# abstractqqq/polars_ds_extension

Measured on AMD Instinct MI355X. Metric: grouped lstsq regressions/sec (1e8 rows x 16 f64 feats; Gram-build GB/s under gram_build), higher is better.
Workload: dtype f64; 1 GPU; group_by(key).agg(lin_reg): 1000000 groups x 100 rows x 16 f64 feats of the frame (1e+08 rows), OLS with rank gate (pl_lr default path), inputs resident in HBM; `value`: the groups given as row offsets (pre-segmented, as Polars hands groups to pl_lr -- the cpu_baseline gets the same); the same step starting from a sorted int64 key column: grouped_by_key; groups_total=1000000, groups_per_gpu=1000000, rows_per_group=100, features=16, parallelism=group-sharded x1

## Files before the change

polars_ds_extension_amd/csrc/grouped_fused.hip:

```cpp
#include <type_traits>

#include "moments_dev.hpp"
#include "solve_reg_dev.hpp"

namespace pds {

#ifdef PDS_PROFILE_PHASES
__device__ unsigned long long g_phase_cycles[8];
#define PDS_T0() const unsigned long long _t0 = __builtin_amdgcn_s_memtime()
#define PDS_T1(k) prof[k] += __builtin_amdgcn_s_memtime() - _t0
#else
#define PDS_T0() do {} while (0)
#define PDS_T1(k) do {} while (0)
#endif

constexpr int kFQ = 18;
constexpr int kFM = kFQ * kFQ;
constexpr int kFTile = 17 * kColStride;
constexpr int kFWaveLds = kFTile + kFM * 8;

template <typename T, bool BIAS>
__device__ __forceinline__ void consume_range(const char* wl, int lane, int rel0, int rel1, WaveAcc& a) {
    const int f = lane & 15, q = lane >> 4;
    const T* xcol = reinterpret_cast<const T*>(wl + f * kColStride) + q;
    const T* ycol = reinterpret_cast<const T*>(wl + kSlotY * kColStride) + q;
    int s0 = rel0 >> 2;
    const int s1 = (rel1 + 3) >> 2;
    using Acc = typename Tile<T>::acc;
    Acc acc;
    double xy, cs, yy, ys;
    if constexpr (sizeof(T) == 8) {
        acc = Acc{a.d[0], a.d[1], a.d[2], a.d[3]};
        xy = a.xy; cs = a.cs; yy = a.yy; ys = a.ys;
    } else {
        acc = Acc{0, 0, 0, 0};
        xy = cs = yy = ys = 0.0;
    }
    T fxy = 0, fcs = 0, fyy = 0, fys = 0;
    auto step_v = [&](T x, T yv) __attribute__((always_inline)) {
        acc = Tile<T>::mfma(x, x, acc);
        if constexpr (sizeof(T) == 8) {
            xy = fma(x, yv, xy);
            if constexpr (BIAS) {
                cs += x;
                ys += yv;
            }
        } else {
            fxy = fmaf(x, yv, fxy);
            if constexpr (BIAS) {
                fcs += x;
                fys += yv;
            }
        }
    };
    auto step = [&](int s, bool masked, int lo, int hi) __attribute__((always_inline)) {
        T x = xcol[4 * s];
        T yv = ycol[4 * s];
        if (masked) {
            const bool in = q >= lo && q < hi;
            x = in ? x : T(0);
            yv = in ? yv : T(0);
        }
        acc = Tile<T>::mfma(x, x, acc);
        if constexpr (sizeof(T) == 8) {
            xy = fma(x, yv, xy);
            if constexpr (BIAS) {
                cs += x;
                ys += yv;
            }
        } else {
            fxy = fmaf(x, yv, fxy);
            if constexpr (BIAS) {
                fcs += x;
                fys += yv;
            }
        }
    };
    if (rel0 & 3) {
        const int lo = rel0 & 3;
        const int hi = min(rel1 - 4 * s0, 4);
        step(s0, true, lo, hi);
        ++s0;
    }
    const int sfull = rel1 >> 2;
    int s = s0;
    for (; s + 4 <= sfull; s += 4) {
        const T x0 = xcol[4 * s], x1 = xcol[4 * s + 4], x2 = xcol[4 * s + 8], x3 = xcol[4 * s + 12];
        const T y0 = ycol[4 * s], y1 = ycol[4 * s + 4], y2 = ycol[4 * s + 8], y3 = ycol[4 * s + 12];
        step_v(x0, y0);
        step_v(x1, y1);
        step_v(x2, y2);
        step_v(x3, y3);
    }
    for (; s < sfull; ++s) step_v(xcol[4 * s], ycol[4 * s]);
    if ((rel1 & 3) && sfull >= s0 && sfull < s1) step(sfull, true, 0, rel1 & 3);
    if constexpr (sizeof(T) == 8) {
        a.d[0] = acc[0]; a.d[1] = acc[1]; a.d[2] = acc[2]; a.d[3] = acc[3];
        a.xy = xy; a.cs = cs; a.yy = yy; a.ys = ys;
    } else {
        a.d[0] += (double)acc[0]; a.d[1] += (double)acc[1]; a.d[2] += (double)acc[2]; a.d[3] += (double)acc[3];
        a.xy += (double)fxy; a.cs += (double)fcs; a.yy += (double)fyy; a.ys += (double)fys;
    }
}

template <typename T, bool BIAS>
__device__ __forceinline__ void consume_range_pack(const char* wl, int lane, int rel0, int rel1, WaveAcc& a) {
    const int f = lane & 15, q = lane >> 4;
    const int roff = q + 4 * (f >> 3);
    const T* xcol = reinterpret_cast<const T*>(wl + (f & 7) * kColStride) + roff;
    const T* ycol = reinterpret_cast<const T*>(wl + kSlotY * kColStride) + roff;
    int s0 = rel0 >> 3;
    const int s1 = (rel1 + 7) >> 3;
    using Acc = typename Tile<T>::acc;
    Acc acc;
    double xy, cs, yy, ys;
    if constexpr (sizeof(T) == 8) {
        acc = Acc{a.d[0], a.d[1], a.d[2], a.d[3]};
        xy = a.xy; cs = a.cs; yy = a.yy; ys = a.ys;
    } else {
        acc = Acc{0, 0, 0, 0};
        xy = cs = yy = ys = 0.0;
    }
    T fxy = 0, fcs = 0, fyy = 0, fys = 0;
    auto step_v = [&](T x, T yv) __attribute__((always_inline)) {
        acc = Tile<T>::mfma(x, x, acc);
        if constexpr (sizeof(T) == 8) {
            xy = fma(x, yv, xy);
            if constexpr (BIAS) {
                cs += x;
                ys += yv;
            }
        } else {
            fxy = fmaf(x, yv, fxy);
            if constexpr (BIAS) {
                fcs += x;
                fys += yv;
            }
        }
    };
    auto step_m = [&](int s) __attribute__((always_inline)) {
        const int r = 8 * s + roff;
        const bool in = r >= rel0 && r < rel1;
        const T x = in ? xcol[8 * s] : T(0);
        const T yv = in ? ycol[8 * s] : T(0);
        step_v(x, yv);
    };
    if (rel0 & 7) {
        step_m(s0);
        ++s0;
    }
    const int sfull = rel1 >> 3;
    int s = s0;
    for (; s + 4 <= sfull; s += 4) {
        const T x0 = xcol[8 * s], x1 = xcol[8 * s + 8], x2 = xcol[8 * s + 16], x3 = xcol[8 * s + 24];
        const T y0 = ycol[8 * s], y1 = ycol[8 * s + 8], y2 = ycol[8 * s + 16], y3 = ycol[8 * s + 24];
        step_v(x0, y0);
        step_v(x1, y1);
        step_v(x2, y2);
        step_v(x3, y3);
    }
    for (; s < sfull; ++s) step_v(xcol[8 * s], ycol[8 * s]);
    if ((rel1 & 7) && sfull >= s0 && sfull < s1) step_m(sfull);
    if constexpr (sizeof(T) == 8) {
        a.d[0] = acc[0]; a.d[1] = acc[1]; a.d[2] = acc[2]; a.d[3] = acc[3];
        a.xy = xy; a.cs = cs; a.yy = yy; a.ys = ys;
    } else {
        a.d[0] += (double)acc[0]; a.d[1] += (double)acc[1]; a.d[2] += (double)acc[2]; a.d[3] += (double)acc[3];
        a.xy += (double)fxy; a.cs += (double)fcs; a.yy += (double)fyy; a.ys += (double)fys;
    }
}

__device__ __forceinline__ int64_t lower_bound_i64(const int64_t* __restrict__ a, int64_t n, int64_t key) {
    int64_t lo = 0, hi = n;
    while (lo < hi) {
        const int64_t mid = (lo + hi) >> 1;
        if (a[mid] < key) lo = mid + 1;
        else hi = mid;
    }
    return lo;
}

template <typename T, int LPS, bool CHOL, bool BIAS, int PC>
__global__ __launch_bounds__(64) void grouped_stream_kernel(const T* const* __restrict__ cols, int p_arg,
                                                            const int64_t* __restrict__ offsets, int64_t n_groups,
                                                            int64_t n_rows, SolveRegDev sp, T* __restrict__ coeffs,
                                                            uint8_t* __restrict__ flags, int32_t* __restrict__ mark_list,
                                                            unsigned* __restrict__ mark_count, unsigned* __restrict__ mark_host_flag) {
    constexpr int SPW = 64 / LPS;
    constexpr int RPL = Tile<T>::RPL;
    constexpr int TR = 64 * RPL;
    constexpr int NA = CHOL ? LPS + 1 : LPS;
    constexpr bool PACK = LPS <= 8;
    constexpr int ZSLOT = PACK ? 7 : 15;
    extern __shared__ __attribute__((aligned(16))) char smem[];
    const int lane = threadIdx.x & 63;
    char* wl = smem;
    double* Msc = reinterpret_cast<double*>(smem + kFTile);
    constexpr bool FULLP = PC != 0;
    static_assert(PC >= 0 && PC <= LPS, "PC is a feature count of this kernel size");
    const int p = FULLP ? PC : p_arg;
    const int pp = p;
    const int pout = p + (BIAS ? 1 : 0);
    const int sub = lane / LPS, j_in = lane % LPS;

    const int64_t W = gridDim.x, w = blockIdx.x;
    const int64_t base_row = offsets[0];
    const int64_t total = offsets[n_groups] - base_row;
    const int64_t gl = (w == 0) ? 0 : lower_bound_i64(offsets, n_groups, base_row + (total * w) / W);
    const int64_t gh = (w == W - 1) ? n_groups : lower_bound_i64(offsets, n_groups, base_row + (total * (w + 1)) / W);
    if (gl >= gh) return;
    const int64_t rlo = offsets[gl], rhi = offsets[gh];

    {
        typename Tile<T>::vec z;
#pragma unroll
        for (int e = 0; e < RPL; ++e) z[e] = T(0);
        for (int c = p; c < 16; ++c) *reinterpret_cast<typename Tile<T>::vec*>(wl + c * kColStride + lane * 16) = z;
    }
#ifdef PDS_PROFILE_PHASES
    unsigned long long prof[8] = {0, 0, 0, 0, 0, 0, 0, 0};
    const unsigned long long t_begin = __builtin_amdgcn_s_memtime();
#endif
    double a_p[NA];
    double b_p[CHOL ? 1 : LPS];
    double dj_p = 1.0;
    double cs_p = 0.0, ys_p = 0.0, n_p = 1.0;
    bool null_p = false;
    int npend = 0;
    int64_t gbase = gl;

    auto solve_pending = [&]() __attribute__((always_inline)) {
        int j = j_in;
        asm volatile("" : "+v"(j));
        const bool colv = j < pp;
        const int64_t sys = gbase + sub;
        const bool live = sub < npend;
        const bool few = null_p;
        bool is_null = null_p;
        bool suspect = false;
        double zj = 0.0;
        int pj = j;
        PDS_T0();
        if constexpr (CHOL) {
            SolveRegDev spk = sp;
            spk.pp = p;
            spk.p = spk.pp;
            spk.gate_on = 1;
            chol_core<LPS>(a_p, dj_p, j, spk, is_null, zj, &suspect);
            suspect = suspect && !few;
            is_null = is_null || suspect;
        } else {
            solve_core<LPS>(a_p, b_p, dj_p, j, lane, sp, is_null, pj, zj);
        }
        if (live && colv) coeffs[sys * (int64_t)pout + pj] = is_null ? (T)__builtin_nan("") : (T)zj;
        if constexpr (BIAS) {
            const double sb = Grp<LPS>::sum(colv ? cs_p * zj : 0.0);
            const double b0 = (ys_p - sb) / n_p;
            if (live && j == 0) coeffs[sys * (int64_t)pout + p] = is_null ? (T)__builtin_nan("") : (T)b0;
        }
        if (live && j == 0 && flags) flags[sys] = suspect ? 2 : (is_null ? 1 : 0);
        if constexpr (CHOL) {
            const bool mk = suspect && live && j == 0;
            const unsigned long long mm = __ballot(mk);
            if (mm != 0ull && mark_list) {
                const int leader = __ffsll((long long)mm) - 1;
                unsigned slot = 0;
                if (lane == leader) {
                    slot = atomicAdd(mark_count, (unsigned)__popcll(mm));
                    __hip_atomic_store(mark_host_flag, 1u, __ATOMIC_RELAXED, __HIP_MEMORY_SCOPE_SYSTEM);
                }
                slot = __shfl(slot, leader);
                if (mk) mark_list[slot + __popcll(mm & ((1ull << lane) - 1ull))] = (int32_t)sys;
            }
        }
        PDS_T1(3);
        gbase += npend;
        npend = 0;
    };

    WaveAcc acc;
    zero_acc(acc);
    int64_t g = gl;
    int64_t gs = rlo;
    int64_t ge = offsets[g + 1];
    uint32_t g_left = (uint32_t)(gh - gl);
    int64_t ge_next = offsets[g_left >= 2 ? g + 2 : gh];
    int64_t pos = rlo;

    auto flush_group = [&]() __attribute__((always_inline)) {
        PDS_T0();
        const uint64_t ng = (uint64_t)(ge - gs);
        const bool too_few = (uint32_t)(ng >> 32) == 0u && (uint32_t)ng < (uint32_t)pout;
        {
            const int jj = lane & 15;
            constexpr bool RFOLD = PACK && sizeof(T) == 8;
            auto shl8 = [](double v) __attribute__((always_inline)) {
                int lo = __double2loint(v), hi = __double2hiint(v);
                lo = __builtin_amdgcn_update_dpp(0, lo, 0x108 , 0xf, 0xf, true);
                hi = __builtin_amdgcn_update_dpp(0, hi, 0x108, 0xf, 0xf, true);
                return __hiloint2double(hi, lo);
            };
            if constexpr (RFOLD) {
                const double d0 = acc.d[0] + shl8(acc.d[2]), d1 = acc.d[1] + shl8(acc.d[3]);
                if (jj < 8) {
                    Msc[Tile<T>::drow(lane, 0) + kFQ * jj] = d0;
                    Msc[Tile<T>::drow(lane, 1) + kFQ * jj] = d1;
                }
            } else {
#pragma unroll
                for (int r = 0; r < 4; ++r) Msc[Tile<T>::drow(lane, r) + kFQ * jj] = acc.d[r];
            }
            double xy = xor_sum_q(acc.xy);
            if constexpr (RFOLD) xy += shl8(xy);
            if (lane < (RFOLD ? 8 : 16)) Msc[lane + kFQ * 17] = xy;
            if constexpr (BIAS) {
                double cs = xor_sum_q(acc.cs), ys = xor_sum_q(acc.ys);
                if constexpr (RFOLD) {
                    cs += shl8(cs);
                    ys += shl8(ys);
                }
                if (lane < (RFOLD ? 8 : 16)) Msc[lane + kFQ * 16] = cs;
                if (lane == 0) {
                    Msc[16 + kFQ * 16] = (double)ng;
                    Msc[16 + kFQ * 17] = ys;
                }
                if (PACK && !RFOLD && lane == 8) Msc[17 + kFQ * 17] = ys;
            }
        }
        if constexpr (PACK && sizeof(T) != 8) {
            PDS_WAVE_LDS_SYNC();
            const int fi = lane & 7, fj = lane >> 3;
            const double dsum = Msc[fi + kFQ * fj] + Msc[fi + 8 + kFQ * (fj + 8)];
            double xys = 0.0, css = 0.0, yss = 0.0;
            if (lane < 8) {
                xys = Msc[lane + kFQ * 17] + Msc[lane + 8 + kFQ * 17];
                if constexpr (BIAS) css = Msc[lane + kFQ * 16] + Msc[lane + 8 + kFQ * 16];
            }
            if (BIAS && lane == 0) yss = Msc[16 + kFQ * 17] + Msc[17 + kFQ * 17];
            PDS_WAVE_LDS_SYNC();
            Msc[fi + kFQ * fj] = dsum;
            if (lane < 8) {
                Msc[lane + kFQ * 17] = xys;
                if constexpr (BIAS) Msc[lane + kFQ * 16] = css;
            }
            if (BIAS && lane == 0) Msc[16 + kFQ * 17] = yss;
        }
        if (sp.lambda > 0.0) {
            PDS_WAVE_LDS_SYNC();
            if (lane < p) Msc[lane * (kFQ + 1)] += sp.lambda;
        }
        PDS_WAVE_LDS_SYNC();
        {
            int j = j_in;
            asm volatile("" : "+v"(j));
            const int lj = (j < p) ? j : ZSLOT;
            if (sub == npend) {
                const double* colp = Msc + kFQ * lj;
                if (p >= LPS) {
#pragma unroll
                    for (int i = 0; i < LPS; ++i) {
                        a_p[i] = colp[i];
                        if constexpr (!CHOL) b_p[i] = Msc[i + kFQ * 17];
                    }
                } else {
#pragma unroll
                    for (int i = 0; i < LPS; ++i) {
                        const int li = (i < p) ? i : ZSLOT;
                        a_p[i] = colp[li];
                        if constexpr (!CHOL) b_p[i] = Msc[li + kFQ * 17];
                    }
                }
                if constexpr (CHOL) a_p[LPS] = Msc[lj + kFQ * 17];
                dj_p = (j < pp) ? colp[lj] : 1.0;
                null_p = too_few;
                if constexpr (BIAS) {
                    static_assert(CHOL, "the centred bias form exists for the Cholesky kernel");
                    const double csj = Msc[lj + kFQ * 16];
                    const double nn = (double)ng, sy = Msc[16 + kFQ * 17];
                    const double m = csj / nn;
#pragma unroll
                    for (int i = 0; i < LPS; ++i) {
                        const int li = (p >= LPS || i < p) ? i : ZSLOT;
                        a_p[i] = fma(-Msc[li + kFQ * 16], m, a_p[i]);
                    }
                    a_p[LPS] = fma(-sy, m, a_p[LPS]);
                    cs_p = csj;
                    ys_p = sy;
                    n_p = nn;
                }
            }
        }
        PDS_WAVE_LDS_SYNC();
        zero_acc(acc);
        ++npend;
        PDS_T1(2);
        if (npend == SPW) solve_pending();
    };

    TileRegs<T> regs;
    const int64_t t_first = rlo / TR, t_last = (rhi > rlo) ? (rhi - 1) / TR : t_first - 1;
    auto load_tile = [&](int64_t t) __attribute__((always_inline)) {
        ColPtrs<T> cp;
#pragma unroll
        for (int c = 0; c < 16; ++c) cp.x[c] = as_global(cols[c]);
        cp.y = as_global(cols[p]);
        cp.w = cp.y;
        const int64_t row = t * TR + lane * RPL;
        if ((t + 1) * TR <= n_rows) load_full_tile<T, false>(cp, p, row, regs);
        else load_tail_tile<T, false>(cp, p, row, n_rows, regs);
    };
    if (t_first <= t_last) load_tile(t_first);
    for (int64_t t = t_first;; ++t) {
        const bool have_tile = t <= t_last;
        if (have_tile) {
            {
                PDS_T0();
                store_tile_lds<T, false>(wl, p, lane, regs);
#ifdef PDS_PROFILE_PHASES
                PDS_WAVE_LDS_SYNC();
#endif
                PDS_T1(0);
            }
            PDS_T0();
            if (t + 1 <= t_last) load_tile(t + 1);
            PDS_T1(1);
        }
        const int64_t row0 = t * TR;
        uint32_t rel_end = 0, pos_rel = 0;
        if (have_tile) {
            const uint64_t left = (uint64_t)(rhi - row0);
            rel_end = ((uint32_t)(left >> 32) != 0u || (uint32_t)left > (uint32_t)TR) ? (uint32_t)TR : (uint32_t)left;
            pos_rel = (uint32_t)(pos - row0);
        }
        auto rel_of = [&](int64_t r) __attribute__((always_inline)) {
            const uint64_t d = (uint64_t)(r - (have_tile ? row0 : pos));
            return ((uint32_t)(d >> 32) != 0u) ? 0xFFFFFFFFu : (uint32_t)d;
        };
        uint32_t ge_rel = rel_of(ge);
        while (g_left != 0u && (pos_rel < rel_end || ge_rel <= pos_rel)) {
            if (ge_rel <= pos_rel) {
                flush_group();
                ++g;
                --g_left;
                gs = ge;
                ge = ge_next;
                ge_next = offsets[g_left >= 2u ? g + 2 : gh];
                ge_rel = rel_of(ge);
                continue;
            }
            const uint32_t seg_end = (ge_rel < rel_end) ? ge_rel : rel_end;
            PDS_T0();
            if constexpr (PACK) consume_range_pack<T, BIAS>(wl, lane, (int)pos_rel, (int)seg_end, acc);
            else consume_range<T, BIAS>(wl, lane, (int)pos_rel, (int)seg_end, acc);
            PDS_T1(4);
            pos_rel = seg_end;
        }
        if (have_tile) pos = row0 + pos_rel;
        if (t >= t_last) break;
        PDS_WAVE_LDS_SYNC();
    }
    if (npend > 0) solve_pending();
#ifdef PDS_PROFILE_PHASES
    prof[7] = __builtin_amdgcn_s_memtime() - t_begin;
    if (lane == 0)
        for (int k = 0; k < 8; ++k) atomicAdd(&g_phase_cycles[k], prof[k]);
#endif
}

template <typename T, int LPS>
static int launch_stream_lps(pds_ctx* ctx, const DeviceCols<T>& dc, int n_feat, const int64_t* d_offsets,
                             int64_t n_groups, int64_t n_rows, const SolveRegDev& sd, bool chol, T* d_coeffs,
                             uint8_t* d_flags, int32_t* d_mark_list, unsigned* d_mark_count, unsigned* d_mark_host) {
    const size_t lds = (size_t)kFWaveLds;
    const int per_cu = std::max(1, (int)((160 * 1024) / lds));
    int64_t nb = std::min<int64_t>(std::max<int64_t>(n_groups / (64 / LPS), 1), (int64_t)ctx->num_cus * per_cu);
    KernelTimer timer(ctx, kKindGroupedMoments);
    if (!chol) return fail(PDS_ERR_INVALID, "internal: fused grouped kernel is Cholesky-only");
    auto go = [&](auto bias_c, auto pc_c) {
        hipLaunchKernelGGL((grouped_stream_kernel<T, LPS, true, decltype(bias_c)::value, decltype(pc_c)::value>), dim3((unsigned)nb),
                           dim3(64), lds, ctx->stream, dc.d_ptrs, n_feat, d_offsets, n_groups, n_rows, sd, d_coeffs, d_flags, d_mark_list,
                           d_mark_count, d_mark_host);
    };
    auto by_pc = [&](auto bias_c) {
        using std::integral_constant;
        constexpr int LO = LPS == 4 ? 1 : LPS / 2 + 1;
        if (n_feat == LPS) return go(bias_c, integral_constant<int, LPS>{});
        if constexpr (sizeof(T) == 8) {
            if (n_feat == LO) return go(bias_c, integral_constant<int, LO>{});
            if constexpr (LPS >= 4) {
                if (n_feat == LO + 1 && LO + 1 < LPS) return go(bias_c, integral_constant<int, (LO + 1 < LPS ? LO + 1 : LPS)>{});
                if (n_feat == LO + 2 && LO + 2 < LPS) return go(bias_c, integral_constant<int, (LO + 2 < LPS ? LO + 2 : LPS)>{});
            }
            if constexpr (LPS == 16) {
                if (n_feat == 12) return go(bias_c, integral_constant<int, 12>{});
                if (n_feat == 13) return go(bias_c, integral_constant<int, 13>{});
                if (n_feat == 14) return go(bias_c, integral_constant<int, 14>{});
                if (n_feat == 15) return go(bias_c, integral_constant<int, 15>{});
            }
        }
        return go(bias_c, integral_constant<int, 0>{});
    };
    if (sd.bias) by_pc(std::true_type{});
    else by_pc(std::false_type{});
    PDS_HIP_CHECK(hipGetLastError());
    return PDS_OK;
}

static int ensure_mark_state(pds_ctx* ctx) {
    if (ctx->mark_count) return PDS_OK;
    PDS_HIP_CHECK(hipMalloc(reinterpret_cast<void**>(&ctx->mark_count), 256));
    ctx->mark_dirty = true;
    PDS_HIP_CHECK(hipHostMalloc(reinterpret_cast<void**>(&ctx->mark_host), 64, hipHostMallocMapped | hipHostMallocCoherent));
    *ctx->mark_host = 0u;
    PDS_HIP_CHECK(hipHostGetDevicePointer(reinterpret_cast<void**>(&ctx->mark_host_dev), ctx->mark_host, 0));
    return PDS_OK;
}

template <typename T>
__global__ void scatter_marked_kernel(const T* __restrict__ co_c, const uint8_t* __restrict__ fl_c, const int32_t* __restrict__ list,
                                      int64_t n, int pp, T* __restrict__ coeffs, uint8_t* __restrict__ flags) {
    const int64_t i = (int64_t)blockIdx.x * blockDim.x + threadIdx.x;
    if (i >= n * pp) return;
    const int64_t k = i / pp;
    const int c = (int)(i - k * pp);
    const int64_t g = list[k];
    coeffs[g * pp + c] = co_c[i];
    if (c == 0) flags[g] = fl_c[k] ? 1 : 0;
}

template <typename T>
int launch_grouped_fused(pds_ctx* ctx, const DeviceCols<T>& dc, int n_feat, int64_t n_rows, const int64_t* d_offsets,
                         int64_t n_groups, const SolveParams& sp, T* d_coeffs, uint8_t* d_flags, T* d_mom_scratch,
                         int64_t scratch_groups) {
    SolveRegDev sd;
    sd.p = sp.p;
    sd.bias = sp.add_bias ? 1 : 0;
    sd.pp = sp.p + sd.bias;
    sd.lambda_on_bias = sp.lambda_on_bias;
    sd.lambda = sp.lambda;
    sd.gate_on = sp.gate_tol > 0.0 ? 1 : 0;
    sd.ln_tol = sd.gate_on ? std::log(sp.gate_tol) : 0.0;
    sd.inv_tol = sd.gate_on ? 1.0 / sp.gate_tol : HUGE_VAL;
    if (n_groups <= 0) return PDS_OK;
    if (n_groups >= (1ll << 31)) return fail(PDS_ERR_INVALID, "internal: fused grouped kernel counts groups per wave in 32 bits");
    const char* piv = dev_env("PDS_GROUPED_PIVOTED");
    const bool chol = sd.gate_on && !(piv && piv[0] == '1');
    const bool second_pass = chol && sp.solver != PDS_SOLVER_CHOLESKEY && d_flags && d_mom_scratch && scratch_groups > 0;
    sd.sus_tol = second_pass ? std::sqrt(sd.inv_tol) : 0.0;
    int32_t* d_list = nullptr;
    unsigned* d_count = nullptr;
    unsigned* d_host = nullptr;
    if (second_pass) {
        if (int rc0 = ensure_mark_state(ctx)) return rc0;
        d_list = reinterpret_cast<int32_t*>(ws_take(ctx, (size_t)n_groups * sizeof(int32_t)));
        if (!d_list) return fail(PDS_ERR_HIP, "workspace allocation failed");
        d_count = ctx->mark_count;
        d_host = ctx->mark_host_dev;
        *ctx->mark_host = 0u;
        if (ctx->mark_dirty) PDS_HIP_CHECK(hipMemsetAsync(d_count, 0, sizeof(unsigned), ctx->stream));
        ctx->mark_dirty = true;
    }
    int rc;
    if (sd.p <= 4) rc = launch_stream_lps<T, 4>(ctx, dc, n_feat, d_offsets, n_groups, n_rows, sd, chol, d_coeffs, d_flags, d_list, d_count, d_host);
    else if (sd.p <= 8) rc = launch_stream_lps<T, 8>(ctx, dc, n_feat, d_offsets, n_groups, n_rows, sd, chol, d_coeffs, d_flags, d_list, d_count, d_host);
    else rc = launch_stream_lps<T, 16>(ctx, dc, n_feat, d_offsets, n_groups, n_rows, sd, chol, d_coeffs, d_flags, d_list, d_count, d_host);
    if (rc || !second_pass) return rc;
    PDS_HIP_CHECK(hipStreamSynchronize(ctx->stream));
    if (__atomic_load_n(ctx->mark_host, __ATOMIC_ACQUIRE) == 0u) {
        ctx->mark_dirty = false;
        return PDS_OK;
    }
    unsigned h_count = 0;
    PDS_HIP_CHECK(hipMemcpyAsync(&h_count, d_count, sizeof(unsigned), hipMemcpyDeviceToHost, ctx->stream));
    PDS_HIP_CHECK(hipMemsetAsync(d_count, 0, sizeof(unsigned), ctx->stream));
    PDS_HIP_CHECK(hipStreamSynchronize(ctx->stream));
    ctx->mark_dirty = false;
    const int64_t marked = (int64_t)h_count;
    if (marked == 0) return PDS_OK;
    const int pp = sd.pp;
    const int64_t chunk = std::min<int64_t>(scratch_groups, marked);
    T* co_c = reinterpret_cast<T*>(ws_take(ctx, (size_t)chunk * pp * sizeof(T)));
    uint8_t* fl_c = reinterpret_cast<uint8_t*>(ws_take(ctx, (size_t)chunk));
    if (!co_c || !fl_c) return fail(PDS_ERR_HIP, "workspace allocation failed");
    for (int64_t k0 = 0; k0 < marked; k0 += chunk) {
        const int64_t kc = std::min(chunk, marked - k0);
        if (int rc2 = launch_grouped_moments<T>(ctx, dc, n_feat, d_offsets, kc, d_mom_scratch, d_list + k0)) return rc2;
        if (int rc2 = launch_solve_marked<T>(ctx, d_mom_scratch, kc, sp, co_c, fl_c, nullptr)) return rc2;
        hipLaunchKernelGGL((scatter_marked_kernel<T>), dim3((unsigned)((kc * pp + 255) / 256)), dim3(256), 0, ctx->stream, co_c, fl_c,
                           d_list + k0, kc, pp, d_coeffs, d_flags);
        PDS_HIP_CHECK(hipGetLastError());
    }
    return PDS_OK;
}

#ifdef PDS_PROFILE_PHASES
extern "C" int pds_debug_phase_cycles(unsigned long long* out, int reset) {
    unsigned long long z[8] = {0, 0, 0, 0, 0, 0, 0, 0};
    if (hipMemcpyFromSymbol(out, HIP_SYMBOL(g_phase_cycles), sizeof(z)) != hipSuccess) return -1;
    if (reset && hipMemcpyToSymbol(HIP_SYMBOL(g_phase_cycles), z, sizeof(z)) != hipSuccess) return -1;
    return 0;
}
#endif

template int launch_grouped_fused<double>(pds_ctx*, const DeviceCols<double>&, int, int64_t, const int64_t*, int64_t,
                                          const SolveParams&, double*, uint8_t*, double*, int64_t);
template int launch_grouped_fused<float>(pds_ctx*, const DeviceCols<float>&, int, int64_t, const int64_t*, int64_t,
                                         const SolveParams&, float*, uint8_t*, float*, int64_t);

}
```

Measured before the change: 394.7 million regressions/s.

## Batch group offset fetches per wave and unify consume_range with remainder prefetch

Merges the packed and unpacked consume_range variants into one templated routine that preloads head, remainder and tail rows before issuing MFMAs, and accumulates directly into a lean GroupAcc without per-call copies. Group end offsets are now fetched 64 at a time into a vector register alongside tile loads and read out with readlane, replacing a dependent scalar global load per group. It also pins occupancy to two waves per EU and restructures the group/segment loop. The aim is to hide offset-load latency and cut per-group overhead with 100-row groups. The cost is more register pressure and a fixed occupancy hint.

```diff
diff --git a/polars_ds_extension_amd/csrc/grouped_fused.hip b/polars_ds_extension_amd/csrc/grouped_fused.hip
--- a/polars_ds_extension_amd/csrc/grouped_fused.hip
+++ b/polars_ds_extension_amd/csrc/grouped_fused.hip
@@ -19,33 +19,35 @@
 constexpr int kFTile = 17 * kColStride;
 constexpr int kFWaveLds = kFTile + kFM * 8;
 
-template <typename T, bool BIAS>
-__device__ __forceinline__ void consume_range(const char* wl, int lane, int rel0, int rel1, WaveAcc& a) {
+struct GroupAcc {
+    d4 d;
+    double xy, cs, ys;
+};
+__device__ __forceinline__ void zero_acc(GroupAcc& a) {
+    a.d = d4{0.0, 0.0, 0.0, 0.0};
+    a.xy = a.cs = a.ys = 0.0;
+}
+
+template <typename T, bool BIAS, bool PACK>
+__device__ __forceinline__ void consume_range(const char* wl, int lane, int rel0, int rel1, GroupAcc& a) {
+    constexpr int SH = PACK ? 3 : 2;
+    constexpr int RS = 1 << SH;
     const int f = lane & 15, q = lane >> 4;
-    const T* xcol = reinterpret_cast<const T*>(wl + f * kColStride) + q;
-    const T* ycol = reinterpret_cast<const T*>(wl + kSlotY * kColStride) + q;
-    int s0 = rel0 >> 2;
-    const int s1 = (rel1 + 3) >> 2;
-    using Acc = typename Tile<T>::acc;
-    Acc acc;
-    double xy, cs, yy, ys;
-    if constexpr (sizeof(T) == 8) {
-        acc = Acc{a.d[0], a.d[1], a.d[2], a.d[3]};
-        xy = a.xy; cs = a.cs; yy = a.yy; ys = a.ys;
-    } else {
-        acc = Acc{0, 0, 0, 0};
-        xy = cs = yy = ys = 0.0;
-    }
-    T fxy = 0, fcs = 0, fyy = 0, fys = 0;
+    const int roff = PACK ? q + 4 * (f >> 3) : q;
+    const T* xcol = reinterpret_cast<const T*>(wl + (PACK ? (f & 7) : f) * kColStride) + roff;
+    const T* ycol = reinterpret_cast<const T*>(wl + kSlotY * kColStride) + roff;
+    f4 facc = {0.f, 0.f, 0.f, 0.f};
+    float fxy = 0, fcs = 0, fys = 0;
     auto step_v = [&](T x, T yv) __attribute__((always_inline)) {
-        acc = Tile<T>::mfma(x, x, acc);
         if constexpr (sizeof(T) == 8) {
-            xy = fma(x, yv, xy);
+            a.d = Tile<T>::mfma(x, x, a.d);
+            a.xy = fma(x, yv, a.xy);
             if constexpr (BIAS) {
-                cs += x;
-                ys += yv;
+                a.cs += x;
+                a.ys += yv;
             }
         } else {
+            facc = Tile<T>::mfma(x, x, facc);
             fxy = fmaf(x, yv, fxy);
             if constexpr (BIAS) {
                 fcs += x;
@@ -53,120 +55,54 @@
             }
         }
     };
-    auto step = [&](int s, bool masked, int lo, int hi) __attribute__((always_inline)) {
-        T x = xcol[4 * s];
-        T yv = ycol[4 * s];
-        if (masked) {
-            const bool in = q >= lo && q < hi;
-            x = in ? x : T(0);
-            yv = in ? yv : T(0);
-        }
-        acc = Tile<T>::mfma(x, x, acc);
-        if constexpr (sizeof(T) == 8) {
-            xy = fma(x, yv, xy);
-            if constexpr (BIAS) {
-                cs += x;
-                ys += yv;
-            }
-        } else {
-            fxy = fmaf(x, yv, fxy);
-            if constexpr (BIAS) {
-                fcs += x;
-                fys += yv;
-            }
-        }
-    };
-    if (rel0 & 3) {
-        const int lo = rel0 & 3;
-        const int hi = min(rel1 - 4 * s0, 4);
-        step(s0, true, lo, hi);
-        ++s0;
-    }
-    const int sfull = rel1 >> 2;
-    int s = s0;
-    for (; s + 4 <= sfull; s += 4) {
-        const T x0 = xcol[4 * s], x1 = xcol[4 * s + 4], x2 = xcol[4 * s + 8], x3 = xcol[4 * s + 12];
-        const T y0 = ycol[4 * s], y1 = ycol[4 * s + 4], y2 = ycol[4 * s + 8], y3 = ycol[4 * s + 12];
+    auto step_m = [&](int s, T x, T yv) __attribute__((always_inline)) {
+        const int r = RS * s + roff;
+        const bool in = r >= rel0 && r < rel1;
+        step_v(in ? x : T(0), in ? yv : T(0));
+    };
+    const int sh = rel0 >> SH;
+    const bool head = (rel0 & (RS - 1)) != 0;
+    const int s0 = sh + (head ? 1 : 0);
+    const int sfull = rel1 >> SH;
+    const bool tail = (rel1 & (RS - 1)) != 0 && sfull >= s0;
+    const int r = sfull > s0 ? ((sfull - s0) & 3) : 0;
+    T xh = 0, yh = 0, xt = 0, yt = 0, xa = 0, ya = 0, xb = 0, yb = 0, xc = 0, yc = 0;
+    if (head) {
+        xh = xcol[RS * sh];
+        yh = ycol[RS * sh];
+    }
+    if (r >= 1) {
+        xa = xcol[RS * s0];
+        ya = ycol[RS * s0];
+    }
+    if (r >= 2) {
+        xb = xcol[RS * s0 + RS];
+        yb = ycol[RS * s0 + RS];
+    }
+    if (r == 3) {
+        xc = xcol[RS * s0 + 2 * RS];
+        yc = ycol[RS * s0 + 2 * RS];
+    }
+    if (tail) {
+        xt = xcol[RS * sfull];
+        yt = ycol[RS * sfull];
+    }
+    if (head) step_m(sh, xh, yh);
+    if (r >= 1) step_v(xa, ya);
+    if (r >= 2) step_v(xb, yb);
+    if (r == 3) step_v(xc, yc);
+    for (int s = s0 + r; s + 4 <= sfull; s += 4) {
+        const T x0 = xcol[RS * s], x1 = xcol[RS * s + RS], x2 = xcol[RS * s + 2 * RS], x3 = xcol[RS * s + 3 * RS];
+        const T y0 = ycol[RS * s], y1 = ycol[RS * s + RS], y2 = ycol[RS * s + 2 * RS], y3 = ycol[RS * s + 3 * RS];
         step_v(x0, y0);
         step_v(x1, y1);
         step_v(x2, y2);
         step_v(x3, y3);
     }
-    for (; s < sfull; ++s) step_v(xcol[4 * s], ycol[4 * s]);
-    if ((rel1 & 3) && sfull >= s0 && sfull < s1) step(sfull, true, 0, rel1 & 3);
-    if constexpr (sizeof(T) == 8) {
-        a.d[0] = acc[0]; a.d[1] = acc[1]; a.d[2] = acc[2]; a.d[3] = acc[3];
-        a.xy = xy; a.cs = cs; a.yy = yy; a.ys = ys;
-    } else {
-        a.d[0] += (double)acc[0]; a.d[1] += (double)acc[1]; a.d[2] += (double)acc[2]; a.d[3] += (double)acc[3];
-        a.xy += (double)fxy; a.cs += (double)fcs; a.yy += (double)fyy; a.ys += (double)fys;
-    }
-}
-
-template <typename T, bool BIAS>
-__device__ __forceinline__ void consume_range_pack(const char* wl, int lane, int rel0, int rel1, WaveAcc& a) {
-    const int f = lane & 15, q = lane >> 4;
-    const int roff = q + 4 * (f >> 3);
-    const T* xcol = reinterpret_cast<const T*>(wl + (f & 7) * kColStride) + roff;
-    const T* ycol = reinterpret_cast<const T*>(wl + kSlotY * kColStride) + roff;
-    int s0 = rel0 >> 3;
-    const int s1 = (rel1 + 7) >> 3;
-    using Acc = typename Tile<T>::acc;
-    Acc acc;
-    double xy, cs, yy, ys;
-    if constexpr (sizeof(T) == 8) {
-        acc = Acc{a.d[0], a.d[1], a.d[2], a.d[3]};
-        xy = a.xy; cs = a.cs; yy = a.yy; ys = a.ys;
-    } else {
-        acc = Acc{0, 0, 0, 0};
-        xy = cs = yy = ys = 0.0;
-    }
-    T fxy = 0, fcs = 0, fyy = 0, fys = 0;
-    auto step_v = [&](T x, T yv) __attribute__((always_inline)) {
-        acc = Tile<T>::mfma(x, x, acc);
-        if constexpr (sizeof(T) == 8) {
-            xy = fma(x, yv, xy);
-            if constexpr (BIAS) {
-                cs += x;
-                ys += yv;
-            }
-        } else {
-            fxy = fmaf(x, yv, fxy);
-            if constexpr (BIAS) {
-                fcs += x;
-                fys += yv;
-            }
-        }
-    };
-    auto step_m = [&](int s) __attribute__((always_inline)) {
-        const int r = 8 * s + roff;
-        const bool in = r >= rel0 && r < rel1;
-        const T x = in ? xcol[8 * s] : T(0);
-        const T yv = in ? ycol[8 * s] : T(0);
-        step_v(x, yv);
-    };
-    if (rel0 & 7) {
-        step_m(s0);
-        ++s0;
-    }
-    const int sfull = rel1 >> 3;
-    int s = s0;
-    for (; s + 4 <= sfull; s += 4) {
-        const T x0 = xcol[8 * s], x1 = xcol[8 * s + 8], x2 = xcol[8 * s + 16], x3 = xcol[8 * s + 24];
-        const T y0 = ycol[8 * s], y1 = ycol[8 * s + 8], y2 = ycol[8 * s + 16], y3 = ycol[8 * s + 24];
-        step_v(x0, y0);
-        step_v(x1, y1);
-        step_v(x2, y2);
-        step_v(x3, y3);
-    }
-    for (; s < sfull; ++s) step_v(xcol[8 * s], ycol[8 * s]);
-    if ((rel1 & 7) && sfull >= s0 && sfull < s1) step_m(sfull);
-    if constexpr (sizeof(T) == 8) {
-        a.d[0] = acc[0]; a.d[1] = acc[1]; a.d[2] = acc[2]; a.d[3] = acc[3];
-        a.xy = xy; a.cs = cs; a.yy = yy; a.ys = ys;
-    } else {
-        a.d[0] += (double)acc[0]; a.d[1] += (double)acc[1]; a.d[2] += (double)acc[2]; a.d[3] += (double)acc[3];
-        a.xy += (double)fxy; a.cs += (double)fcs; a.yy += (double)fyy; a.ys += (double)fys;
+    if (tail) step_m(sfull, xt, yt);
+    if constexpr (sizeof(T) != 8) {
+        a.d[0] += (double)facc[0]; a.d[1] += (double)facc[1]; a.d[2] += (double)facc[2]; a.d[3] += (double)facc[3];
+        a.xy += (double)fxy; a.cs += (double)fcs; a.ys += (double)fys;
     }
 }
 
@@ -181,7 +117,7 @@
 }
 
 template <typename T, int LPS, bool CHOL, bool BIAS, int PC>
-__global__ __launch_bounds__(64) void grouped_stream_kernel(const T* const* __restrict__ cols, int p_arg,
+__global__ __launch_bounds__(64) __attribute__((amdgpu_waves_per_eu(2, 2))) void grouped_stream_kernel(const T* const* __restrict__ cols, int p_arg,
                                                             const int64_t* __restrict__ offsets, int64_t n_groups,
                                                             int64_t n_rows, SolveRegDev sp, T* __restrict__ coeffs,
                                                             uint8_t* __restrict__ flags, int32_t* __restrict__ mark_list,
@@ -278,13 +214,31 @@
         npend = 0;
     };
 
-    WaveAcc acc;
+    GroupAcc acc;
     zero_acc(acc);
-    int64_t g = gl;
+    int32_t g = (int32_t)gl;
+    int64_t blk = 0, blk_n = 0;
+    int32_t gblk = g - 64, gblk_n = g - 64;
+    auto fetch_block = [&](int32_t g0) __attribute__((always_inline)) {
+        const int64_t i = (int64_t)g0 + lane;
+        return as_global(offsets)[i < n_groups ? i : n_groups];
+    };
+    auto end_of = [&](int32_t gi) __attribute__((always_inline)) {
+        int idx = gi + 1 - gblk;
+        if (idx >= 64) {
+            blk = fetch_block(gi);
+            asm volatile("" : "+v"(blk));
+            gblk = gi;
+            idx = 1;
+        }
+        idx = __builtin_amdgcn_readfirstlane(idx);
+        const uint32_t lo = (uint32_t)__builtin_amdgcn_readlane((int)(uint32_t)blk, idx);
+        const uint32_t hi = (uint32_t)__builtin_amdgcn_readlane((int)(uint32_t)((uint64_t)blk >> 32), idx);
+        return (int64_t)(((uint64_t)hi << 32) | lo);
+    };
     int64_t gs = rlo;
     int64_t ge = offsets[g + 1];
     uint32_t g_left = (uint32_t)(gh - gl);
-    int64_t ge_next = offsets[g_left >= 2 ? g + 2 : gh];
     int64_t pos = rlo;
 
     auto flush_group = [&]() __attribute__((always_inline)) {
@@ -406,6 +360,8 @@
         cp.y = as_global(cols[p]);
         cp.w = cp.y;
         const int64_t row = t * TR + lane * RPL;
+        blk_n = fetch_block(g);
+        gblk_n = g;
         if ((t + 1) * TR <= n_rows) load_full_tile<T, false>(cp, p, row, regs);
         else load_tail_tile<T, false>(cp, p, row, n_rows, regs);
     };
@@ -416,6 +372,9 @@
             {
                 PDS_T0();
                 store_tile_lds<T, false>(wl, p, lane, regs);
+                blk = blk_n;
+                gblk = gblk_n;
+                asm volatile("" : "+v"(blk) : : "memory");
 #ifdef PDS_PROFILE_PHASES
                 PDS_WAVE_LDS_SYNC();
 #endif
@@ -437,23 +396,22 @@
             return ((uint32_t)(d >> 32) != 0u) ? 0xFFFFFFFFu : (uint32_t)d;
         };
         uint32_t ge_rel = rel_of(ge);
-        while (g_left != 0u && (pos_rel < rel_end || ge_rel <= pos_rel)) {
-            if (ge_rel <= pos_rel) {
-                flush_group();
-                ++g;
-                --g_left;
-                gs = ge;
-                ge = ge_next;
-                ge_next = offsets[g_left >= 2u ? g + 2 : gh];
-                ge_rel = rel_of(ge);
-                continue;
-            }
-            const uint32_t seg_end = (ge_rel < rel_end) ? ge_rel : rel_end;
-            PDS_T0();
-            if constexpr (PACK) consume_range_pack<T, BIAS>(wl, lane, (int)pos_rel, (int)seg_end, acc);
-            else consume_range<T, BIAS>(wl, lane, (int)pos_rel, (int)seg_end, acc);
-            PDS_T1(4);
-            pos_rel = seg_end;
+        while (g_left != 0u) {
+            if (pos_rel < ge_rel) {
+                if (pos_rel >= rel_end) break;
+                const uint32_t seg_end = (ge_rel < rel_end) ? ge_rel : rel_end;
+                PDS_T0();
+                consume_range<T, BIAS, PACK>(wl, lane, (int)pos_rel, (int)seg_end, acc);
+                PDS_T1(4);
+                pos_rel = seg_end;
+                if (pos_rel < ge_rel) break;
+            }
+            flush_group();
+            ++g;
+            --g_left;
+            gs = ge;
+            if (g_left != 0u) ge = end_of(g);
+            ge_rel = rel_of(ge);
         }
         if (have_tile) pos = row0 + pos_rel;
         if (t >= t_last) break;
```

Measured after the change: 398.6 million regressions/s (median of 6 runs). No clear change (+1.0%).

## Split fused grouped kernel into producer/solver wave pairs with LDS ring handoff

Applied to the files above, without the earlier changes.

For the 16-lane Cholesky path with a fixed feature count, each 512-thread workgroup now runs four streaming waves that build Gram moments and four solver waves that solve them. The two sides pass groups through a two-slot LDS ring guarded by sequence flags and s_sleep polling. This lets the Gram accumulation overlap with the per-group Cholesky solve instead of running them back to back in one wave. The cost is a large LDS footprint (about 80 KB per workgroup) and spin-wait synchronisation. There is also a new failure path if the device will not grant that much dynamic LDS.

```diff
diff --git a/polars_ds_extension_amd/csrc/grouped_fused.hip b/polars_ds_extension_amd/csrc/grouped_fused.hip
--- a/polars_ds_extension_amd/csrc/grouped_fused.hip
+++ b/polars_ds_extension_amd/csrc/grouped_fused.hip
@@ -6,7 +6,7 @@
 namespace pds {
 
 #ifdef PDS_PROFILE_PHASES
-__device__ unsigned long long g_phase_cycles[8];
+__device__ unsigned long long g_phase_cycles[16];
 #define PDS_T0() const unsigned long long _t0 = __builtin_amdgcn_s_memtime()
 #define PDS_T1(k) prof[k] += __builtin_amdgcn_s_memtime() - _t0
 #else
@@ -18,6 +18,18 @@
 constexpr int kFM = kFQ * kFQ;
 constexpr int kFTile = 17 * kColStride;
 constexpr int kFWaveLds = kFTile + kFM * 8;
+
+#ifndef PDS_GROUPED_FUSED_PAIRED
+#define PDS_GROUPED_FUSED_PAIRED 1
+#endif
+constexpr int kFSlotTri = 136, kFSlotXY = kFSlotTri, kFSlotCS = kFSlotXY + 16, kFSlotN = kFSlotCS + 16, kFSlotYS = kFSlotN + 1,
+              kFSlotGid = kFSlotYS + 1, kFSlotFew = kFSlotGid + 1, kFSlotDoubles = kFSlotFew + 1;
+constexpr int kFSlots = 2, kFSlotBytes = kFSlotDoubles * 8;
+constexpr int kFPairLds = 2800;
+constexpr int kFPairedLds = 4 * kFTile + 4 * kFPairLds;
+static_assert(kFSlotDoubles == 172 && kFSlots * kFSlotBytes + 12 <= kFPairLds, "two slots and three words per pair");
+static_assert(2 * kFPairedLds <= 160 * 1024, "two workgroups per CU");
+__host__ __device__ constexpr int fslot_tri(int i) { return (i * (31 - i)) / 2; }
 
 template <typename T, bool BIAS>
 __device__ __forceinline__ void consume_range(const char* wl, int lane, int rel0, int rel1, WaveAcc& a) {
@@ -180,12 +192,12 @@
     return lo;
 }
 
-template <typename T, int LPS, bool CHOL, bool BIAS, int PC>
-__global__ __launch_bounds__(64) void grouped_stream_kernel(const T* const* __restrict__ cols, int p_arg,
-                                                            const int64_t* __restrict__ offsets, int64_t n_groups,
-                                                            int64_t n_rows, SolveRegDev sp, T* __restrict__ coeffs,
-                                                            uint8_t* __restrict__ flags, int32_t* __restrict__ mark_list,
-                                                            unsigned* __restrict__ mark_count, unsigned* __restrict__ mark_host_flag) {
+template <typename T, int LPS, bool CHOL, bool BIAS, int PC, bool PAIRED = false>
+__global__ __attribute__((amdgpu_flat_work_group_size(1, PAIRED ? 512 : 64), amdgpu_waves_per_eu(PAIRED ? 4 : 0)))
+void grouped_stream_kernel(const T* const* __restrict__ cols, int p_arg, const int64_t* __restrict__ offsets, int64_t n_groups,
+                           int64_t n_rows, SolveRegDev sp, T* __restrict__ coeffs, uint8_t* __restrict__ flags,
+                           int32_t* __restrict__ mark_list, unsigned* __restrict__ mark_count, unsigned* __restrict__ mark_host_flag) {
+    static_assert(!PAIRED || (LPS == 16 && CHOL), "the paired form exists for the 16-lane Cholesky kernel");
     constexpr int SPW = 64 / LPS;
     constexpr int RPL = Tile<T>::RPL;
     constexpr int TR = 64 * RPL;
@@ -194,8 +206,15 @@
     constexpr int ZSLOT = PACK ? 7 : 15;
     extern __shared__ __attribute__((aligned(16))) char smem[];
     const int lane = threadIdx.x & 63;
-    char* wl = smem;
+    const int wv = PAIRED ? __builtin_amdgcn_readfirstlane((int)(threadIdx.x >> 6)) : 0, pairi = wv & 3;
+    const bool solver = PAIRED && wv >= 4;
+    char* wl = smem + (PAIRED ? pairi * kFTile : 0);
     double* Msc = reinterpret_cast<double*>(smem + kFTile);
+    typedef __attribute__((address_space(3))) char* lds_c;
+    typedef __attribute__((address_space(3))) double* lds_dp;
+    typedef volatile __attribute__((address_space(3))) unsigned* lds_flag;
+    const lds_c ring = (lds_c)smem + 4 * kFTile + pairi * kFPairLds;
+    const lds_flag FL = (lds_flag)(ring + kFSlots * kFSlotBytes);
     constexpr bool FULLP = PC != 0;
     static_assert(PC >= 0 && PC <= LPS, "PC is a feature count of this kernel size");
     const int p = FULLP ? PC : p_arg;
@@ -203,29 +222,32 @@
     const int pout = p + (BIAS ? 1 : 0);
     const int sub = lane / LPS, j_in = lane % LPS;
 
-    const int64_t W = gridDim.x, w = blockIdx.x;
-    const int64_t base_row = offsets[0];
-    const int64_t total = offsets[n_groups] - base_row;
-    const int64_t gl = (w == 0) ? 0 : lower_bound_i64(offsets, n_groups, base_row + (total * w) / W);
-    const int64_t gh = (w == W - 1) ? n_groups : lower_bound_i64(offsets, n_groups, base_row + (total * (w + 1)) / W);
-    if (gl >= gh) return;
-    const int64_t rlo = offsets[gl], rhi = offsets[gh];
-
-    {
-        typename Tile<T>::vec z;
-#pragma unroll
-        for (int e = 0; e < RPL; ++e) z[e] = T(0);
-        for (int c = p; c < 16; ++c) *reinterpret_cast<typename Tile<T>::vec*>(wl + c * kColStride + lane * 16) = z;
+    if constexpr (PAIRED) {
+        if (!solver && lane < 3) FL[lane] = 0u;
+        __syncthreads();
     }
 #ifdef PDS_PROFILE_PHASES
-    unsigned long long prof[8] = {0, 0, 0, 0, 0, 0, 0, 0};
+    unsigned long long prof[16] = {0, 0, 0, 0, 0, 0, 0, 0, 0, 0, 0, 0, 0, 0, 0, 0};
     const unsigned long long t_begin = __builtin_amdgcn_s_memtime();
 #endif
+    const int64_t W = PAIRED ? (int64_t)gridDim.x * 4 : (int64_t)gridDim.x, w = PAIRED ? (int64_t)blockIdx.x * 4 + pairi : (int64_t)blockIdx.x;
+    int64_t gl = 0, gh = 0;
+    if (!solver) {
+        const int64_t base_row = offsets[0];
+        const int64_t total = offsets[n_groups] - base_row;
+        gl = (w == 0) ? 0 : lower_bound_i64(offsets, n_groups, base_row + (total * w) / W);
+        gh = (w == W - 1) ? n_groups : lower_bound_i64(offsets, n_groups, base_row + (total * (w + 1)) / W);
+        if (gl >= gh) {
+            if constexpr (PAIRED) FL[2] = 1u;
+            return;
+        }
+    }
     double a_p[NA];
     double b_p[CHOL ? 1 : LPS];
     double dj_p = 1.0;
     double cs_p = 0.0, ys_p = 0.0, n_p = 1.0;
     bool null_p = false;
+    int few_p = 0, gid_lo = 0, gid_hi = 0;
     int npend = 0;
     int64_t gbase = gl;
 
@@ -233,7 +255,8 @@
         int j = j_in;
         asm volatile("" : "+v"(j));
         const bool colv = j < pp;
-        const int64_t sys = gbase + sub;
+        if constexpr (PAIRED) null_p = few_p != 0;
+        const int64_t sys = PAIRED ? (int64_t)(((uint64_t)(uint32_t)gid_hi << 32) | (uint64_t)(uint32_t)gid_lo) : gbase + sub;
         const bool live = sub < npend;
         const bool few = null_p;
         bool is_null = null_p;
@@ -273,11 +296,132 @@
                 if (mk) mark_list[slot + __popcll(mm & ((1ull << lane) - 1ull))] = (int32_t)sys;
             }
         }
-        PDS_T1(3);
+        PDS_T1(PAIRED ? 11 : 3);
         gbase += npend;
         npend = 0;
     };
 
+    if constexpr (PAIRED) {
+        if (solver) {
+            unsigned cseq = 0;
+            auto wait_group = [&]() __attribute__((always_inline)) {
+                PDS_T0();
+                bool got;
+                for (;;) {
+                    const unsigned dv = FL[2], fv = FL[0];
+                    const unsigned d = (unsigned)__builtin_amdgcn_readfirstlane((int)dv), f = (unsigned)__builtin_amdgcn_readfirstlane((int)fv);
+                    if (f != cseq) {
+                        got = true;
+                        break;
+                    }
+                    if (d) {
+                        got = false;
+                        break;
+                    }
+                    __builtin_amdgcn_s_sleep(2);
+                }
+                asm volatile("" ::: "memory");
+                PDS_T1(8);
+                return got;
+            };
+            auto take = [&](auto rm) __attribute__((always_inline)) {
+                constexpr int ROW = decltype(rm)::value;
+                PDS_T0();
+                const lds_dp S = (lds_dp)(ring + (int)(cseq & (kFSlots - 1)) * kFSlotBytes);
+                if (sp.lambda > 0.0) {
+                    if (lane < p) S[fslot_tri(lane) + lane] += sp.lambda;
+                    PDS_WAVE_LDS_SYNC();
+                }
+                auto put = [&](double& dst, double v) __attribute__((always_inline)) {
+                    if constexpr (ROW == 0) dst = v;
+                    else dst = __builtin_amdgcn_update_dpp(dst, v, 0xE4 , 1 << ROW, 0xf, false);
+                };
+                auto puti = [&](int& dst, int v) __attribute__((always_inline)) {
+                    if constexpr (ROW == 0) dst = v;
+                    else dst = __builtin_amdgcn_update_dpp(dst, v, 0xE4, 1 << ROW, 0xf, false);
+                };
+                int j = j_in;
+                asm volatile("" : "+v"(j));
+                const int lj = (j < p) ? j : ZSLOT;
+                int colb = lj, rowb = fslot_tri(lj);
+                asm volatile("" : "+v"(colb), "+v"(rowb));
+                double vxy = S[kFSlotXY + colb];
+                const double diag = S[rowb + colb];
+                const double djv = (j < pp) ? diag : 1.0;
+                const __attribute__((address_space(3))) int* Si = (const __attribute__((address_space(3))) int*)S;
+                const int glo = Si[2 * kFSlotGid], ghi = Si[2 * kFSlotGid + 1], fw = Si[2 * kFSlotFew];
+                double m = 0.0;
+                if constexpr (BIAS) {
+                    const double csj = S[kFSlotCS + colb];
+                    const double nn = S[kFSlotN], sy = S[kFSlotYS];
+                    m = csj / nn;
+                    vxy = fma(-sy, m, vxy);
+                    put(cs_p, csj);
+                    put(ys_p, sy);
+                    put(n_p, nn);
+                }
+                put(a_p[LPS], vxy);
+                put(dj_p, djv);
+#pragma unroll
+                for (int b = 0; b < LPS; b += 8) {
+                    double v[8];
+#pragma unroll
+                    for (int k = 0; k < 8; ++k) {
+                        const int i = b + k, li = (i < p) ? i : ZSLOT;
+                        v[k] = S[(li <= lj) ? fslot_tri(li) + colb : rowb + li];
+                        if constexpr (BIAS) v[k] = fma(-S[kFSlotCS + li], m, v[k]);
+                    }
+#pragma unroll
+                    for (int k = 0; k < 8; ++k) put(a_p[b + k], v[k]);
+                    __builtin_amdgcn_sched_barrier(0);
+                }
+                puti(gid_lo, glo);
+                puti(gid_hi, ghi);
+                puti(few_p, fw);
+                PDS_WAVE_LDS_SYNC();
+                ++cseq;
+                FL[1] = cseq;
+                PDS_T1(9);
+            };
+            using std::integral_constant;
+            for (;;) {
+                npend = 0;
+                if (wait_group()) {
+                    take(integral_constant<int, 0>{});
+                    npend = 1;
+                    if (wait_group()) {
+                        take(integral_constant<int, 1>{});
+                        npend = 2;
+                        if (wait_group()) {
+                            take(integral_constant<int, 2>{});
+                            npend = 3;
+                            if (wait_group()) {
+                                take(integral_constant<int, 3>{});
+                                npend = 4;
+                            }
+                        }
+                    }
+                }
+                const bool last = npend < SPW;
+                if (npend > 0) solve_pending();
+                if (last) break;
+            }
+#ifdef PDS_PROFILE_PHASES
+            prof[15] = __builtin_amdgcn_s_memtime() - t_begin;
+            if (lane == 0)
+                for (int k = 8; k < 16; ++k) atomicAdd(&g_phase_cycles[k], prof[k]);
+#endif
+            return;
+        }
+    }
+    const int64_t rlo = offsets[gl], rhi = offsets[gh];
+
+    {
+        typename Tile<T>::vec z;
+#pragma unroll
+        for (int e = 0; e < RPL; ++e) z[e] = T(0);
+        for (int c = p; c < 16; ++c) *reinterpret_cast<typename Tile<T>::vec*>(wl + c * kColStride + lane * 16) = z;
+    }
     WaveAcc acc;
     zero_acc(acc);
     int64_t g = gl;
@@ -286,11 +430,50 @@
     uint32_t g_left = (uint32_t)(gh - gl);
     int64_t ge_next = offsets[g_left >= 2 ? g + 2 : gh];
     int64_t pos = rlo;
+    unsigned pseq = 0;
 
     auto flush_group = [&]() __attribute__((always_inline)) {
-        PDS_T0();
         const uint64_t ng = (uint64_t)(ge - gs);
         const bool too_few = (uint32_t)(ng >> 32) == 0u && (uint32_t)ng < (uint32_t)pout;
+        if constexpr (PAIRED) {
+            {
+                PDS_T0();
+                while ((unsigned)((int)pseq - __builtin_amdgcn_readfirstlane((int)FL[1])) >= (unsigned)kFSlots) __builtin_amdgcn_s_sleep(1);
+                asm volatile("" ::: "memory");
+                PDS_T1(5);
+            }
+            PDS_T0();
+            const lds_dp S = (lds_dp)(ring + (int)(pseq & (kFSlots - 1)) * kFSlotBytes);
+            int ln = lane;
+            asm volatile("" : "+v"(ln));
+            const int jj = ln & 15;
+#pragma unroll
+            for (int r = 0; r < 4; ++r) {
+                const int i = Tile<T>::drow(ln, r);
+                if (i <= jj) S[fslot_tri(i) + jj] = acc.d[r];
+            }
+            const double xy = xor_sum_q(acc.xy);
+            if (ln < 16) S[kFSlotXY + ln] = xy;
+            if constexpr (BIAS) {
+                const double cs = xor_sum_q(acc.cs), ys = xor_sum_q(acc.ys);
+                if (ln < 16) S[kFSlotCS + ln] = cs;
+                if (ln == 0) {
+                    S[kFSlotN] = (double)ng;
+                    S[kFSlotYS] = ys;
+                }
+            }
+            if (ln == 0) {
+                S[kFSlotGid] = __longlong_as_double((long long)g);
+                S[kFSlotFew] = __longlong_as_double(too_few ? 1ll : 0ll);
+            }
+            PDS_WAVE_LDS_SYNC();
+            ++pseq;
+            FL[0] = pseq;
+            zero_acc(acc);
+            PDS_T1(2);
+            return;
+        }
+        PDS_T0();
         {
             const int jj = lane & 15;
             constexpr bool RFOLD = PACK && sizeof(T) == 8;
@@ -459,7 +642,12 @@
         if (t >= t_last) break;
         PDS_WAVE_LDS_SYNC();
     }
-    if (npend > 0) solve_pending();
+    if constexpr (PAIRED) {
+        PDS_WAVE_LDS_SYNC();
+        FL[2] = 1u;
+    } else {
+        if (npend > 0) solve_pending();
+    }
 #ifdef PDS_PROFILE_PHASES
     prof[7] = __builtin_amdgcn_s_memtime() - t_begin;
     if (lane == 0)
@@ -476,10 +664,24 @@
     int64_t nb = std::min<int64_t>(std::max<int64_t>(n_groups / (64 / LPS), 1), (int64_t)ctx->num_cus * per_cu);
     KernelTimer timer(ctx, kKindGroupedMoments);
     if (!chol) return fail(PDS_ERR_INVALID, "internal: fused grouped kernel is Cholesky-only");
+    constexpr bool kPaired = LPS == 16 && PDS_GROUPED_FUSED_PAIRED != 0;
+    int attr_rc = PDS_OK;
     auto go = [&](auto bias_c, auto pc_c) {
-        hipLaunchKernelGGL((grouped_stream_kernel<T, LPS, true, decltype(bias_c)::value, decltype(pc_c)::value>), dim3((unsigned)nb),
-                           dim3(64), lds, ctx->stream, dc.d_ptrs, n_feat, d_offsets, n_groups, n_rows, sd, d_coeffs, d_flags, d_mark_list,
-                           d_mark_count, d_mark_host);
+        if constexpr (kPaired && decltype(pc_c)::value != 0) {
+            auto kern = grouped_stream_kernel<T, LPS, true, decltype(bias_c)::value, decltype(pc_c)::value, true>;
+            if (hipFuncSetAttribute(reinterpret_cast<const void*>(kern), hipFuncAttributeMaxDynamicSharedMemorySize, kFPairedLds) != hipSuccess) {
+                (void)hipGetLastError();
+                attr_rc = fail(PDS_ERR_HIP, "fused grouped kernel: the device does not grant a workgroup 80 KB of LDS");
+                return;
+            }
+            const int64_t nsw = std::min<int64_t>(std::max<int64_t>(n_groups / (64 / LPS), 1), (int64_t)ctx->num_cus * 8);
+            hipLaunchKernelGGL(kern, dim3((unsigned)((nsw + 3) / 4)), dim3(512), (size_t)kFPairedLds, ctx->stream, dc.d_ptrs, n_feat, d_offsets,
+                               n_groups, n_rows, sd, d_coeffs, d_flags, d_mark_list, d_mark_count, d_mark_host);
+        } else {
+            hipLaunchKernelGGL((grouped_stream_kernel<T, LPS, true, decltype(bias_c)::value, decltype(pc_c)::value>), dim3((unsigned)nb),
+                               dim3(64), lds, ctx->stream, dc.d_ptrs, n_feat, d_offsets, n_groups, n_rows, sd, d_coeffs, d_flags, d_mark_list,
+                               d_mark_count, d_mark_host);
+        }
     };
     auto by_pc = [&](auto bias_c) {
         using std::integral_constant;
@@ -502,6 +704,7 @@
     };
     if (sd.bias) by_pc(std::true_type{});
     else by_pc(std::false_type{});
+    if (attr_rc) return attr_rc;
     PDS_HIP_CHECK(hipGetLastError());
     return PDS_OK;
 }
@@ -595,7 +798,7 @@
 
 #ifdef PDS_PROFILE_PHASES
 extern "C" int pds_debug_phase_cycles(unsigned long long* out, int reset) {
-    unsigned long long z[8] = {0, 0, 0, 0, 0, 0, 0, 0};
+    unsigned long long z[16] = {0, 0, 0, 0, 0, 0, 0, 0, 0, 0, 0, 0, 0, 0, 0, 0};
     if (hipMemcpyFromSymbol(out, HIP_SYMBOL(g_phase_cycles), sizeof(z)) != hipSuccess) return -1;
     if (reset && hipMemcpyToSymbol(HIP_SYMBOL(g_phase_cycles), z, sizeof(z)) != hipSuccess) return -1;
     return 0;
```

Measured after the change: 404.5 million regressions/s before, 394.4 million regressions/s after. -2.5%, worse.
